# arpitbansal297/Cold-Diffusion-Models

Measured on NVIDIA H100. Metric: training-step images/sec (CelebA-128 deblur UNet, config 3), higher is better.
Workload: dtype tf32

## Files before the change

### cold_diffusion_models_b200/_lib.py

```python
import ctypes as C
import os
import torch

_HERE = os.path.dirname(os.path.abspath(__file__))
LIB_PATH = os.path.join(_HERE, 'csrc', 'libcolddiff.so')
CD_MAX_TAPS = 16
CONV_SIMT, CONV_TC = 0, 1
ACT_NONE, ACT_GELU, ACT_GELU_BWD = 0, 1, 2


class ColdDiffError(RuntimeError):
    pass


if not os.path.exists(LIB_PATH):
    raise ImportError("libcolddiff.so not built (%s); run `python -c 'import __graft_entry__ as g; g.build()'`"
                      % LIB_PATH)
lib = C.CDLL(LIB_PATH)


class ConvSrc(C.Structure):
    _fields_ = [('src', C.c_void_p), ('ld', C.c_int32), ('C', C.c_int32), ('H', C.c_int32), ('W', C.c_int32),
                ('ntaps', C.c_int32), ('dy', C.c_int32 * CD_MAX_TAPS), ('dx', C.c_int32 * CD_MAX_TAPS),
                ('w', C.c_void_p), ('w_per_batch', C.c_int32)]


class ConvDesc(C.Structure):
    _fields_ = [('B', C.c_int32), ('Hg', C.c_int32), ('Wg', C.c_int32), ('sy', C.c_int32), ('sx', C.c_int32),
                ('Cout', C.c_int32), ('nsrc', C.c_int32), ('s', ConvSrc * 2),
                ('out', C.c_void_p), ('out_ld', C.c_int32), ('Ho', C.c_int32), ('Wo', C.c_int32),
                ('oys', C.c_int32), ('oxs', C.c_int32), ('oy0', C.c_int32), ('ox0', C.c_int32),
                ('bias', C.c_void_p), ('resid', C.c_void_p), ('resid_ld', C.c_int32),
                ('act', C.c_int32), ('round_tf32', C.c_int32),
                ('out2', C.c_void_p), ('out2_ld', C.c_int32),
                ('aux', C.c_void_p), ('aux_ld', C.c_int32)]




class RepackJob(C.Structure):
    _fields_ = [('src', C.c_void_p), ('dst', C.c_void_p), ('O', C.c_int32), ('I', C.c_int32), ('KH', C.c_int32), ('KW', C.c_int32),
                ('transposed_conv', C.c_int32), ('mode', C.c_int32), ('ntaps', C.c_int32), ('round_tf32', C.c_int32),
                ('ky', C.c_int32 * CD_MAX_TAPS), ('kx', C.c_int32 * CD_MAX_TAPS), ('block0', C.c_int32), ('nblocks', C.c_int32)]


lib.cd_version.restype = C.c_int
if os.environ.get('COLDDIFF_2CTA') in ('0', '1', '2'):
    lib.cd_conv_tc_set_2cta(int(os.environ['COLDDIFF_2CTA']))
lib.cd_last_error.argtypes = [C.c_char_p, C.c_size_t]
if os.environ.get('COLDDIFF_CONV_TWO_CTAS') in ('0', '64', '128', '192'):
    lib.cd_conv_tc_set_two_ctas(int(os.environ['COLDDIFF_CONV_TWO_CTAS']))
if os.environ.get('COLDDIFF_CONV_HALO') in ('0', '1', '2', '6', '8'):
    lib.cd_conv_tc_set_halo(int(os.environ['COLDDIFF_CONV_HALO']))
if os.environ.get('COLDDIFF_WGRAD_MODE') in ('0', '1', '8'):
    lib.cd_wgrad_tc_set_mode(int(os.environ['COLDDIFF_WGRAD_MODE']))
if os.environ.get('COLDDIFF_2CTA_BN') in ('0', '64', '128', '192'):
    lib.cd_conv_tc_set_2cta_bn(int(os.environ['COLDDIFF_2CTA_BN']))
if os.environ.get('COLDDIFF_CONV_STAGED_EPILOGUE') in ('0', '1', '2', '3'):
    lib.cd_conv_tc_set_staged_epilogue(int(os.environ['COLDDIFF_CONV_STAGED_EPILOGUE']))
if os.environ.get('COLDDIFF_CONV_SIMT_PRELOAD') in ('0', '1'):
    lib.cd_conv_simt_set_preload(int(os.environ['COLDDIFF_CONV_SIMT_PRELOAD']))
if os.environ.get('COLDDIFF_LAYERNORM_MULTI') in ('0', '2', '4'):
    lib.cd_layernorm_set_multi(int(os.environ['COLDDIFF_LAYERNORM_MULTI']))
if os.environ.get('COLDDIFF_LINATTN_STAGED') in ('0', '1'):
    lib.cd_linattn_set_staged(int(os.environ['COLDDIFF_LINATTN_STAGED']))


def _check(rc, what):
    if rc != 0:
        buf = C.create_string_buffer(512)
        lib.cd_last_error(buf, 512)
        raise ColdDiffError("%s failed (%d): %s" % (what, rc, buf.value.decode()))


def stream():
    return C.c_void_p(torch.cuda.current_stream().cuda_stream)


def ptr(t):
    if t is None:
        return C.c_void_p(0)
    return C.c_void_p(t.data_ptr())


_LAUNCHES = {'cd_linattn_context': 2, 'cd_linattn_context_det': 2, 'cd_conv_wgrad': 2, 'cd_time_mlp_fwd': 2, 'cd_time_mlp2_fwd': 2, 'cd_version': 0, 'cd_last_error': 0}
_launch_count = 0


_PROF_SHAPE_ARGS = {'cd_dwconv7_fwd': (2, 3, 4, 5), 'cd_dwconv7_wgrad': (4, 5, 6, 7), 'cd_layernorm_bwd': (6, 7),
                    'cd_layernorm_fwd': (2, 3), 'cd_linattn_context': (2, 3), 'cd_linattn_context_det': (2, 3), 'cd_linattn_bwd_kv': (2, 3)}
_prof = None


def call(name, *args):
    global _launch_count
    _launch_count += _LAUNCHES.get(name, 1)
    if _prof is not None:
        e0, e1 = torch.cuda.Event(enable_timing=True), torch.cuda.Event(enable_timing=True)
        e0.record()
        _check(getattr(lib, name)(*args), name)
        e1.record()
        idx = _PROF_SHAPE_ARGS.get(name)
        if idx:
            name = name + str(tuple(int(getattr(args[i], 'value', args[i])) for i in idx))
        _prof.append((name, e0, e1))
        return
    _check(getattr(lib, name)(*args), name)


def profile_start():
    global _prof
    _prof = []


def profile_stop():
    global _prof
    torch.cuda.synchronize()
    out = {}
    for name, e0, e1 in _prof:
        c, t = out.get(name, (0, 0.0))
        out[name] = (c + 1, t + e0.elapsed_time(e1))
    _prof = None
    return out


def reset_launch_count():
    global _launch_count
    _launch_count = 0


def launch_count():
    return _launch_count


EXPORTS = [
    'cd_version', 'cd_last_error', 'cd_conv_fwd', 'cd_conv_wgrad', 'cd_pack_weight', 'cd_unpack_wgrad',
]
```

### cold_diffusion_models_b200/csrc/conv_tc.cu

```cuda
#include "tc_common.cuh"
#include "conv_epilogue.cuh"

namespace {

constexpr int kTileM = 128;
constexpr int kChunkK = 32;
constexpr int kABytes = kTileM * 128;
constexpr int kThreads = 288;
constexpr int kConsumerWarps = 8;

struct TcParams {
  int B, Hg, Wg;
  int TW, TH, TN;
  int tiles_x, tiles_y, tiles_n, tiles_co, total_tiles;
  int sy, sx;
  int Cout;
  int nsrc;
  int ntaps[2];
  int kchunks[2];
  int wpb[2];
  int8_t dy[2][CD_MAX_TAPS];
  int8_t dx[2][CD_MAX_TAPS];
  float* out; int out_ld; int Ho, Wo; int oys, oxs, oy0, ox0;
  const float* bias;
  const float* resid; int resid_ld;
  int act; int round_tf32;
  float* out2; int out2_ld;
  const float* aux; int aux_ld;
  int nbox[2];
  int8_t boxdx[2][3];
  int8_t boxend[2][3];
  int8_t taporder[2][CD_MAX_TAPS];
  int tapoff[2][CD_MAX_TAPS];
};

__device__ __forceinline__ long long tile_pixel(const TcParams& p, int tile, int m) {
  int mt = tile / p.tiles_co;
  const int tx = mt % p.tiles_x; mt /= p.tiles_x;
  const int ty = mt % p.tiles_y;
  const int tn = mt / p.tiles_y;
  const int gx = tx * p.TW + m % p.TW, gy = ty * p.TH + (m / p.TW) % p.TH, b = tn * p.TN + m / (p.TW * p.TH);
  if (b >= p.B) return -1;
  return (static_cast<long long>(b) * p.Ho + (gy * p.oys + p.oy0)) * p.Wo + (gx * p.oxs + p.ox0);
}

__device__ __forceinline__ void epi_pair(const TcParams& p, long long pix, int col, float v0, float v1) {
  if (col + 1 < p.Cout) {
    float2 v = make_float2(v0, v1);
    if (p.bias) { const float2 b = __ldg(reinterpret_cast<const float2*>(p.bias + col)); v.x += b.x; v.y += b.y; }
    if (p.resid) { const float2 r = *reinterpret_cast<const float2*>(p.resid + pix * p.resid_ld + col); v.x += r.x; v.y += r.y; }
    if (p.out2) *reinterpret_cast<float2*>(p.out2 + pix * p.out2_ld + col) = v;
    if (p.act == CD_ACT_GELU) { v.x = cd_gelu(v.x); v.y = cd_gelu(v.y); }
    else if (p.act == CD_ACT_GELU_BWD) {
      const float2 a = *reinterpret_cast<const float2*>(p.aux + pix * p.aux_ld + col);
      v.x *= cd_gelu_grad(a.x); v.y *= cd_gelu_grad(a.y);
    }
    if (p.round_tf32) { v.x = cd_round_tf32(v.x); v.y = cd_round_tf32(v.y); }
    *reinterpret_cast<float2*>(p.out + pix * p.out_ld + col) = v;
  } else if (col < p.Cout) {
    float v = v0;
    if (p.bias) v += p.bias[col];
    if (p.resid) v += p.resid[pix * p.resid_ld + col];
    if (p.out2) p.out2[pix * p.out2_ld + col] = v;
    if (p.act == CD_ACT_GELU) v = cd_gelu(v);
    else if (p.act == CD_ACT_GELU_BWD) v *= cd_gelu_grad(p.aux[pix * p.aux_ld + col]);
    if (p.round_tf32) v = cd_round_tf32(v);
    p.out[pix * p.out_ld + col] = v;
  }
}

template <int BN, int STAGES, bool STG = false, bool F16 = false, int CTAS = 1, bool PAIR = false>
__global__ void __launch_bounds__(kThreads, CTAS)
conv_tc_kernel(const __grid_constant__ CUtensorMap mapA0, const __grid_constant__ CUtensorMap mapA1,
               const __grid_constant__ CUtensorMap mapB0, const __grid_constant__ CUtensorMap mapB1,
               const TcParams p) {
  constexpr int kBBytes = BN * 128;
  constexpr int kStageBytes = kABytes + kBBytes;
  constexpr int kChunkElems = F16 ? 64 : kChunkK;

  extern __shared__ uint8_t smem_raw[];
  const uint32_t raw_addr = smem_u32(smem_raw);
  const uint32_t pad = (1024u - (raw_addr & 1023u)) & 1023u;
  uint8_t* smem = smem_raw + pad;
  uint64_t* bars = reinterpret_cast<uint64_t*>(smem + STAGES * kStageBytes);
  uint64_t* full_bar = bars;
  uint64_t* empty_bar = bars + STAGES;
  static_assert(2 * STAGES * 8 <= 256, "barrier block is 256 bytes");
  float* epi_stage = reinterpret_cast<float*>(smem + STAGES * kStageBytes + 256);

  const int warp = threadIdx.x >> 5;
  const int lane = threadIdx.x & 31;
  const int wg = threadIdx.x >> 7;

  if (threadIdx.x == 0) {
    for (int i = 0; i < STAGES; ++i) { mbar_init(&full_bar[i], 1); mbar_init(&empty_bar[i], kConsumerWarps * (PAIR ? 2 : 1)); }
    asm volatile("fence.mbarrier_init.release.cluster;" ::: "memory");
  }
  if constexpr (PAIR) cluster_sync(); else __syncthreads();
  const uint32_t rank = PAIR ? cluster_ctarank() : 0;
  const int unit0 = PAIR ? blockIdx.x / 2 : blockIdx.x, ustride = PAIR ? gridDim.x / 2 : gridDim.x;
  const int units = PAIR ? p.tiles_co * ((p.total_tiles / p.tiles_co + 1) / 2) : p.total_tiles;
  auto tile_of = [&](int u) { return PAIR ? ((u / p.tiles_co) * 2 + static_cast<int>(rank)) * p.tiles_co + u % p.tiles_co : u; };

  const int kiters = p.ntaps[0] * p.kchunks[0] + (p.nsrc > 1 ? p.ntaps[1] * p.kchunks[1] : 0);

  if (warp == kConsumerWarps) {
    if (elect_one()) {
      uint32_t stage = 0, ph = 0;
      for (int u = unit0; u < units; u += ustride) {
        const int tile = tile_of(u);
        const int co_t = tile % p.tiles_co;
        int mt = tile / p.tiles_co;
        const int tx = mt % p.tiles_x; mt /= p.tiles_x;
        const int ty = mt % p.tiles_y;
        const int tn = mt / p.tiles_y;
        const int x0 = tx * p.TW * p.sx, y0 = ty * p.TH * p.sy, n0 = tn * p.TN, co0 = co_t * BN;
        for (int s = 0; s < p.nsrc; ++s) {
          const CUtensorMap* mA = s ? &mapA1 : &mapA0;
          const CUtensorMap* mB = s ? &mapB1 : &mapB0;
          const int wbase = p.wpb[s] ? n0 * p.ntaps[s] : 0;
          for (int tap = 0; tap < p.ntaps[s]; ++tap) {
            const int xin = x0 + p.dx[s][tap], yin = y0 + p.dy[s][tap];
            for (int kc = 0; kc < p.kchunks[s]; ++kc) {
              mbar_wait(&empty_bar[stage], ph ^ 1u);
              mbar_expect_tx(&full_bar[stage], kStageBytes);
              const uint32_t sa = smem_u32(smem + stage * kStageBytes);
              tma_load_4d(sa, mA, &full_bar[stage], kc * kChunkElems, xin, yin, n0);
              if constexpr (PAIR)
                tma_load_3d_mc(sa + kABytes + rank * (kBBytes / 2), mB, &full_bar[stage], kc * kChunkElems, co0 + static_cast<int>(rank) * (BN / 2),
                               wbase + tap, static_cast<uint16_t>(3));
              else
                tma_load_3d(sa + kABytes, mB, &full_bar[stage], kc * kChunkElems, co0, wbase + tap);
              if (++stage == STAGES) { stage = 0; ph ^= 1u; }
            }
          }
        }
      }
    }
    __syncwarp();
  } else {
    const int cw = wg;
    const int tid = threadIdx.x & 127;
    const int rl = (tid >> 5) * 16 + (lane >> 2);
    const int q2 = (lane & 3) * 2;
    float acc[BN / 2];
    uint32_t stage = 0, ph = 0;
    auto release = [&](uint32_t st) {
      __syncwarp();
      if (lane == 0) { mbar_arrive(&empty_bar[st]); if constexpr (PAIR) mbar_arrive_cluster(&empty_bar[st], rank ^ 1u); }
    };
    for (int u = unit0; u < units; u += ustride) {
      const int tile = tile_of(u);
      uint32_t prev = 0;
      for (int k = 0; k < kiters; ++k) {
        mbar_wait(&full_bar[stage], ph);
        wgmma_fence();
        const uint32_t sa = smem_u32(smem + stage * kStageBytes);
        const uint64_t da = make_kmajor_sw128_desc(sa + cw * (kABytes / 2));
        const uint64_t db = make_kmajor_sw128_desc(sa + kABytes);
#pragma unroll
        for (int kk = 0; kk < 4; ++kk) {
          if constexpr (F16) wgmma_f16<BN>(acc, da + uint64_t(kk * 2), db + uint64_t(kk * 2), (k | kk) != 0 ? 1u : 0u);
          else wgmma_tf32<BN>(acc, da + uint64_t(kk * 2), db + uint64_t(kk * 2), (k | kk) != 0 ? 1u : 0u);
        }
        wgmma_commit();
        wgmma_wait<1>();
        if (k > 0) release(prev);
        prev = stage;
        if (++stage == STAGES) { stage = 0; ph ^= 1u; }
      }
      wgmma_wait<0>();
      if (kiters > 0) release(prev);

      const int co0 = (tile % p.tiles_co) * BN;
      const long long pix0 = tile_pixel(p, tile, cw * 64 + rl);
      const long long pix1 = tile_pixel(p, tile, cw * 64 + rl + 8);
      if constexpr (STG) {
        float* st = epi_stage + cw * 64 * kEpiStageStride;
        const int bar_id = 1 + cw;
#pragma unroll
        for (int c = 0; c < BN; c += 32) {
          if (co0 + c + 32 <= p.Cout) {
            asm volatile("bar.sync %0, 128;" :: "r"(bar_id) : "memory");
#pragma unroll
            for (int j = c / 8; j < c / 8 + 4; ++j) {
              *reinterpret_cast<float2*>(st + rl * kEpiStageStride + 8 * j - c + q2) = make_float2(acc[4 * j], acc[4 * j + 1]);
              *reinterpret_cast<float2*>(st + (rl + 8) * kEpiStageStride + 8 * j - c + q2) = make_float2(acc[4 * j + 2], acc[4 * j + 3]);
            }
            asm volatile("bar.sync %0, 128;" :: "r"(bar_id) : "memory");
            const int w4 = tid >> 5;
            if (w4 < 2) {
              const int row = w4 * 32 + lane;
              uint32_t r[32];
#pragma unroll
              for (int e = 0; e < 32; ++e) r[e] = __float_as_uint(st[row * kEpiStageStride + e]);
              const long long pix = tile_pixel(p, tile, cw * 64 + row);
              cd_epilogue_staged32(r, st + w4 * 32 * kEpiStageStride, lane, pix < 0 ? 0 : pix, pix >= 0, co0 + c, p);
            }
          } else {
#pragma unroll
            for (int j = c / 8; j < c / 8 + 4; ++j) {
              if (pix0 >= 0) epi_pair(p, pix0, co0 + 8 * j + q2, acc[4 * j], acc[4 * j + 1]);
              if (pix1 >= 0) epi_pair(p, pix1, co0 + 8 * j + q2, acc[4 * j + 2], acc[4 * j + 3]);
            }
          }
        }
      } else {
#pragma unroll
        for (int j = 0; j < BN / 8; ++j) {
          if (pix0 >= 0) epi_pair(p, pix0, co0 + 8 * j + q2, acc[4 * j], acc[4 * j + 1]);
          if (pix1 >= 0) epi_pair(p, pix1, co0 + 8 * j + q2, acc[4 * j + 2], acc[4 * j + 3]);
        }
      }
    }
  }
  if constexpr (PAIR) cluster_sync();
}

constexpr int kRowsTW = 16, kRowsTH = kTileM / kRowsTW;
constexpr int kRowsBoxBytes = kRowsTW * (kRowsTH + 2) * 128;

template <int BN, int ABOXES, int STAGES, int CTAS>
__global__ void __launch_bounds__(kThreads, CTAS)
conv_rows_kernel(const __grid_constant__ CUtensorMap mapA0, const __grid_constant__ CUtensorMap mapA1,
                 const __grid_constant__ CUtensorMap mapB0, const __grid_constant__ CUtensorMap mapB1, const __grid_constant__ TcParams p) {
  constexpr int kBBytes = BN * 128;
  extern __shared__ uint8_t smem_raw[];
  const uint32_t raw_addr = smem_u32(smem_raw);
  uint8_t* smem = smem_raw + ((1024u - (raw_addr & 1023u)) & 1023u);
  uint8_t* abox = smem;
  uint8_t* wtile = smem + ABOXES * kRowsBoxBytes;
  uint64_t* bars = reinterpret_cast<uint64_t*>(wtile + STAGES * kBBytes);
  uint64_t* full_bar = bars;
  uint64_t* empty_bar = bars + STAGES;
  uint64_t* afull = bars + 2 * STAGES;
  uint64_t* aempty = bars + 2 * STAGES + ABOXES;
  static_assert(2 * (STAGES + ABOXES) * 8 <= 256, "barrier block is 256 bytes");
  const int warp = threadIdx.x >> 5, lane = threadIdx.x & 31, wg = threadIdx.x >> 7;
  if (threadIdx.x == 0) {
    for (int i = 0; i < STAGES; ++i) { mbar_init(&full_bar[i], 1); mbar_init(&empty_bar[i], kConsumerWarps); }
    for (int i = 0; i < ABOXES; ++i) { mbar_init(&afull[i], 1); mbar_init(&aempty[i], kConsumerWarps); }
    asm volatile("fence.mbarrier_init.release.cluster;" ::: "memory");
  }
  __syncthreads();

  if (warp == kConsumerWarps) {
    if (elect_one()) {
      uint32_t stage = 0, ph = 0, ai = 0, aph = 0;
      for (int tile = blockIdx.x; tile < p.total_tiles; tile += gridDim.x) {
        const int co0 = (tile % p.tiles_co) * BN;
        int mt = tile / p.tiles_co;
        const int x0 = (mt % p.tiles_x) * kRowsTW; mt /= p.tiles_x;
        const int y0 = (mt % p.tiles_y) * kRowsTH;
        const int n = mt / p.tiles_y;
        for (int s = 0; s < p.nsrc; ++s) {
          const CUtensorMap* mA = s ? &mapA1 : &mapA0;
          const CUtensorMap* mB = s ? &mapB1 : &mapB0;
          for (int kc = 0; kc < p.kchunks[s]; ++kc) {
            for (int b = 0, i = 0; b < p.nbox[s]; ++b) {
              mbar_wait(&aempty[ai], aph ^ 1u);
              mbar_expect_tx(&afull[ai], kRowsBoxBytes);
              tma_load_4d(smem_u32(abox + ai * kRowsBoxBytes), mA, &afull[ai], kc * kChunkK, x0 + p.boxdx[s][b], y0 - 1, n);
              if (++ai == ABOXES) { ai = 0; aph ^= 1u; }
              for (; i < p.boxend[s][b]; ++i) {
                mbar_wait(&empty_bar[stage], ph ^ 1u);
                mbar_expect_tx(&full_bar[stage], kBBytes);
                tma_load_3d(smem_u32(wtile + stage * kBBytes), mB, &full_bar[stage], kc * kChunkK, co0, p.taporder[s][i]);
                if (++stage == STAGES) { stage = 0; ph ^= 1u; }
              }
            }
          }
        }
      }
    }
    __syncwarp();
    return;
  }

  const int tid = threadIdx.x & 127;
  const int rl = (tid >> 5) * 16 + (lane >> 2);
  const int q2 = (lane & 3) * 2;
  auto release = [&](uint64_t* bar) { __syncwarp(); if (lane == 0) mbar_arrive(bar); };
  float acc[BN / 2];
  uint32_t stage = 0, ph = 0, ai = 0, aph = 0;
  for (int tile = blockIdx.x; tile < p.total_tiles; tile += gridDim.x) {
    int k = 0;
    uint32_t prev = 0, prev_a = 0;
    for (int s = 0; s < p.nsrc; ++s) {
      for (int kc = 0; kc < p.kchunks[s]; ++kc) {
        for (int b = 0, i = 0; b < p.nbox[s]; ++b) {
          mbar_wait(&afull[ai], aph);
          const uint32_t abase = smem_u32(abox + ai * kRowsBoxBytes) + wg * (kABytes / 2);
          for (const int i0 = i; i < p.boxend[s][b]; ++i, ++k) {
            mbar_wait(&full_bar[stage], ph);
            wgmma_fence();
            const uint64_t da = make_kmajor_sw128_desc(abase + p.tapoff[s][i]);
            const uint64_t db = make_kmajor_sw128_desc(smem_u32(wtile + stage * kBBytes));
#pragma unroll
            for (int kk = 0; kk < 4; ++kk)
              wgmma_tf32<BN>(acc, da + uint64_t(kk * 2), db + uint64_t(kk * 2), (k | kk) != 0 ? 1u : 0u);
            wgmma_commit();
            wgmma_wait<1>();
            if (k > 0) release(&empty_bar[prev]);
            if (k > 0 && i == i0) release(&aempty[prev_a]);
            prev = stage;
            if (++stage == STAGES) { stage = 0; ph ^= 1u; }
          }
          prev_a = ai;
          if (++ai == ABOXES) { ai = 0; aph ^= 1u; }
        }
      }
    }
    wgmma_wait<0>();
    if (k > 0) { release(&empty_bar[prev]); release(&aempty[prev_a]); }

    const int co0 = (tile % p.tiles_co) * BN;
    int mt = tile / p.tiles_co;
    const int x0 = (mt % p.tiles_x) * kRowsTW; mt /= p.tiles_x;
    const int y0 = (mt % p.tiles_y) * kRowsTH;
    const int n = mt / p.tiles_y;
#pragma unroll
    for (int h = 0; h < 2; ++h) {
      const int m = wg * 64 + rl + 8 * h;
      const int gx = x0 + m % kRowsTW, gy = y0 + m / kRowsTW;
      if (gx >= p.Wg || gy >= p.Hg) continue;
      const long long pix = (static_cast<long long>(n) * p.Ho + (gy * p.oys + p.oy0)) * p.Wo + (gx * p.oxs + p.ox0);
#pragma unroll
      for (int j = 0; j < BN / 8; ++j) epi_pair(p, pix, co0 + 8 * j + q2, acc[4 * j + 2 * h], acc[4 * j + 2 * h + 1]);
    }
  }
}


int g_num_sms = 0;
int g_tf32_map_dtype = 1;


template <int BN, int STAGES, bool STG = false, bool F16 = false, int CTAS = 1, bool PAIR = false>
int launch(const CUtensorMap* maps, const TcParams& p, cudaStream_t st) {
  constexpr size_t smem = size_t(STAGES) * (kABytes + BN * 128) + 1024 + 256 + (STG ? sizeof(float) * 2 * 64 * kEpiStageStride : 0);
  static_assert(smem <= 232448, "dynamic shared memory of one CTA (227 KB)");
  static_assert(CTAS == 1 || 2 * (smem + 1024) <= 233472, "two CTAs per SM must fit the 228 KB of shared memory");
  auto kern = conv_tc_kernel<BN, STAGES, STG, F16, CTAS, PAIR>;
  static bool attr_done = false;
  if (!attr_done) {
    CD_CUDA(cudaFuncSetAttribute(kern, cudaFuncAttributeMaxDynamicSharedMemorySize, (int)smem));
    attr_done = true;
  }
  if constexpr (PAIR) {
    const int units = p.tiles_co * ((p.total_tiles / p.tiles_co + 1) / 2), slots = g_num_sms / 2;
    cudaLaunchConfig_t cfg = {};
    cudaLaunchAttribute attr[1];
    attr[0].id = cudaLaunchAttributeClusterDimension;
    attr[0].val.clusterDim.x = 2; attr[0].val.clusterDim.y = 1; attr[0].val.clusterDim.z = 1;
    cfg.gridDim = dim3(2 * (units < slots ? units : slots)); cfg.blockDim = dim3(kThreads);
    cfg.dynamicSmemBytes = smem; cfg.stream = st; cfg.attrs = attr; cfg.numAttrs = 1;
    CD_CUDA(cudaLaunchKernelEx(&cfg, kern, maps[0], maps[1], maps[2], maps[3], p));
  } else {
    const int slots = g_num_sms * CTAS;
    const int grid = p.total_tiles < slots ? p.total_tiles : slots;
    kern<<<grid, kThreads, smem, st>>>(maps[0], maps[1], maps[2], maps[3], p);
  }
  CD_LAUNCH_CHECK();
  return 0;
}

template <int BN, int ABOXES, int STAGES, int CTAS = 1>
int launch_rows(const CUtensorMap* maps, const TcParams& p, cudaStream_t st) {
  constexpr size_t smem = size_t(ABOXES) * kRowsBoxBytes + size_t(STAGES) * BN * 128 + 1024 + 256;
  static_assert(smem <= 232448, "dynamic shared memory of one CTA (227 KB)");
  static_assert(CTAS == 1 || 2 * (smem + 1024) <= 233472, "two CTAs per SM must fit the 228 KB of shared memory");
  auto kern = conv_rows_kernel<BN, ABOXES, STAGES, CTAS>;
  static bool attr_done = false;
  if (!attr_done) {
    CD_CUDA(cudaFuncSetAttribute(kern, cudaFuncAttributeMaxDynamicSharedMemorySize, (int)smem));
    attr_done = true;
  }
  const int slots = g_num_sms * CTAS;
  const int grid = p.total_tiles < slots ? p.total_tiles : slots;
  kern<<<grid, kThreads, smem, st>>>(maps[0], maps[1], maps[2], maps[3], p);
  CD_LAUNCH_CHECK();
  return 0;
}

}

extern "C" int cd_conv_tc_set_tf32_maps(int enable) { g_tf32_map_dtype = enable ? 1 : 0; return 0; }

static int g_use_2cta = 0;
extern "C" int cd_conv_tc_set_2cta(int mode) { g_use_2cta = mode; return 0; }
static int g_2cta_bn = 0;
extern "C" int cd_conv_tc_set_2cta_bn(int mask) { g_2cta_bn = mask & (128 | 64); return 0; }
static int g_use_halo = 0;
extern "C" int cd_conv_tc_set_halo(int enable) { g_use_halo = enable; return 0; }
static int g_ctas2 = 128 | 64;
extern "C" int cd_conv_tc_set_two_ctas(int mask) { g_ctas2 = mask & (128 | 64); return 0; }
static int g_epi_staged = 0;
constexpr int kStagedMaxKIters = 16;
constexpr int kStagedMidKIters = 48;
extern "C" int cd_conv_tc_set_staged_epilogue(int mode) { g_epi_staged = mode; return 0; }

static double tc_cost(long long m_tiles, int Cout, int BN, int sms, bool pair = false) {
  if (pair) {
    const long long tiles = ((m_tiles + 1) / 2) * (Cout / 256), slots = sms / 2;
    return double((tiles + slots - 1) / slots) * 256.0;
  }
  const long long tiles = m_tiles * ((Cout + BN - 1) / BN);
  const double rate = BN == 256 ? 0.92 : (BN == 128 ? 0.75 : 0.40);
  return double((tiles + sms - 1) / sms) * BN / rate;
}

static int conv_fwd_tc_impl(const CdConvDesc* d, cudaStream_t st, bool f16);
int cd_conv_fwd_tc(const CdConvDesc* d, cudaStream_t st) { return conv_fwd_tc_impl(d, st, false); }

extern "C" int cd_conv_fwd_f16_probe(const CdConvDesc* d, void* stream) {
  CD_REQUIRE(d != nullptr && d->nsrc >= 1 && d->nsrc <= 2, "cd_conv_fwd_f16_probe: bad descriptor");
  return conv_fwd_tc_impl(d, static_cast<cudaStream_t>(stream), true);
}

static int conv_fwd_rows(const CdConvDesc* d, cudaStream_t st, bool by_shape);

static int conv_fwd_tc_impl(const CdConvDesc* d, cudaStream_t st, bool f16) {
  if (!f16 && g_epi_staged == 0) {
    if ((g_use_halo == 0 && !g_use_2cta) || g_use_halo == 1 || g_use_halo == 2 || g_use_halo == 6) {
      const int r = conv_fwd_rows(d, st, g_use_halo == 0);
      if (r <= 0) return r;
    }
  }
  const int chunk_elems = f16 ? 64 : kChunkK;
  const int esz = f16 ? 2 : 4;
  EncodeTiledFn enc = get_encode();
  CD_REQUIRE(enc != nullptr, "cuTensorMapEncodeTiled entry point unavailable");
  if (!g_num_sms) {
    int dev = 0; CD_CUDA(cudaGetDevice(&dev));
    CD_CUDA(cudaDeviceGetAttribute(&g_num_sms, cudaDevAttrMultiProcessorCount, dev));
  }
  CD_REQUIRE(d->nsrc >= 1 && d->nsrc <= 2, "conv_tc: nsrc must be 1 or 2");
  TcParams p{};
  p.B = d->B; p.Hg = d->Hg; p.Wg = d->Wg; p.sy = d->sy; p.sx = d->sx; p.Cout = d->Cout; p.nsrc = d->nsrc;
  if (d->Wg >= 128) {
    CD_REQUIRE(d->Wg % 128 == 0, "conv_tc: Wg >= 128 must be a multiple of 128 (got %d)", d->Wg);
    p.TW = 128; p.TH = 1; p.TN = 1;
  } else {
    CD_REQUIRE(is_pow2(d->Wg), "conv_tc: Wg < 128 must be a power of two (got %d)", d->Wg);
    p.TW = d->Wg;
    int th = 128 / p.TW;
    if (th > d->Hg) th = d->Hg;
    CD_REQUIRE(is_pow2(th) && d->Hg % th == 0, "conv_tc: unsupported Hg %d for Wg %d", d->Hg, d->Wg);
    p.TH = th; p.TN = 128 / (p.TW * p.TH);
  }
  CD_REQUIRE(p.TW * d->sx <= 256 && p.TH * d->sy <= 256, "conv_tc: strided box too large");
  p.tiles_x = d->Wg / p.TW; p.tiles_y = d->Hg / p.TH; p.tiles_n = cd_cdiv(d->B, p.TN);
  int BN = (d->Cout % 256 == 0) ? 256 : (d->Cout > 64 ? 128 : 64);
  int kiters_host = 0;
  for (int s = 0; s < d->nsrc; ++s) kiters_host += d->s[s].ntaps * (d->s[s].C / chunk_elems);
  const bool staged = !f16 &&
                      ( g_epi_staged == 2 || (g_epi_staged == 1 && kiters_host <= kStagedMaxKIters) ||
                      (g_epi_staged == 3 && kiters_host <= kStagedMidKIters));
  bool pair = false;
  const long long mt = static_cast<long long>(p.tiles_x) * p.tiles_y * p.tiles_n;
  if (BN == 256) {
    double best = tc_cost(mt, d->Cout, 256, g_num_sms);
    if (tc_cost(mt, d->Cout, 128, g_num_sms) < best) { BN = 128; best = tc_cost(mt, d->Cout, 128, g_num_sms); }
    if (!f16 && !staged && g_use_2cta && mt >= 2 && (g_use_2cta == 2 || tc_cost(mt, d->Cout, 256, g_num_sms, true) < best)) {
      BN = 256; pair = true;
    }
  } else if (!f16 && !staged && g_use_2cta && (g_2cta_bn & BN) && d->Cout % BN == 0 && (g_use_2cta == 2 || mt >= 2 * g_num_sms)) {
    pair = true;
  }
  p.tiles_co = cd_cdiv(d->Cout, BN);
  p.total_tiles = p.tiles_x * p.tiles_y * p.tiles_n * p.tiles_co;
  p.out = d->out; p.out_ld = d->out_ld; p.Ho = d->Ho; p.Wo = d->Wo;
  p.oys = d->oys; p.oxs = d->oxs; p.oy0 = d->oy0; p.ox0 = d->ox0;
  p.bias = d->bias; p.resid = d->resid; p.resid_ld = d->resid_ld; p.act = d->act; p.round_tf32 = d->round_tf32;
  p.out2 = d->out2; p.out2_ld = d->out2_ld; p.aux = d->aux; p.aux_ld = d->aux_ld;
  CD_REQUIRE(d->act != CD_ACT_GELU_BWD || (d->aux && (reinterpret_cast<uintptr_t>(d->aux) & 15) == 0 && d->aux_ld % 4 == 0), "conv_tc: GELU_BWD needs an aligned aux");
  CD_REQUIRE((reinterpret_cast<uintptr_t>(d->out) & 15) == 0 && d->out_ld % 4 == 0, "conv_tc: out must be 16B aligned");
  CD_REQUIRE(!d->resid || ((reinterpret_cast<uintptr_t>(d->resid) & 15) == 0 && d->resid_ld % 4 == 0), "conv_tc: resid alignment");
  CD_REQUIRE(!d->out2 || ((reinterpret_cast<uintptr_t>(d->out2) & 15) == 0 && d->out2_ld % 4 == 0), "conv_tc: out2 alignment");
  CD_REQUIRE(!d->bias || (reinterpret_cast<uintptr_t>(d->bias) & 15) == 0, "conv_tc: bias alignment");

  CUtensorMap maps[4];
  const CUtensorMapDataType dt = f16 ? CU_TENSOR_MAP_DATA_TYPE_FLOAT16 : (g_tf32_map_dtype ? CU_TENSOR_MAP_DATA_TYPE_TFLOAT32 : CU_TENSOR_MAP_DATA_TYPE_FLOAT32);
  for (int s = 0; s < 2; ++s) {
    const CdConvSrc& cs = d->s[s < d->nsrc ? s : 0];
    CD_REQUIRE(cs.C % chunk_elems == 0 && cs.C > 0, "conv_tc: source channels %d not a multiple of %d", cs.C, chunk_elems);
    CD_REQUIRE(cs.ntaps >= 1 && cs.ntaps <= CD_MAX_TAPS, "conv_tc: bad ntaps");
    CD_REQUIRE((reinterpret_cast<uintptr_t>(cs.src) & 15) == 0 && (cs.ld * esz) % 16 == 0, "conv_tc: src must be 16B aligned");
    CD_REQUIRE((reinterpret_cast<uintptr_t>(cs.w) & 15) == 0, "conv_tc: weights must be 16B aligned");
    CD_REQUIRE(!cs.w_per_batch || p.TN == 1, "conv_tc: per-batch weights need >=128 pixels per image");
    p.ntaps[s] = cs.ntaps; p.kchunks[s] = cs.C / chunk_elems; p.wpb[s] = cs.w_per_batch;
    for (int t = 0; t < cs.ntaps; ++t) { p.dy[s][t] = (int8_t)cs.dy[t]; p.dx[s][t] = (int8_t)cs.dx[t]; }
    {
      cuuint64_t dims[4] = {(cuuint64_t)cs.C, (cuuint64_t)cs.W, (cuuint64_t)cs.H, (cuuint64_t)d->B};
      cuuint64_t strides[3] = {(cuuint64_t)cs.ld * esz, (cuuint64_t)cs.ld * esz * cs.W, (cuuint64_t)cs.ld * esz * cs.W * cs.H};
      cuuint32_t box[4] = {(cuuint32_t)chunk_elems, (cuuint32_t)(p.TW * d->sx), (cuuint32_t)(p.TH * d->sy), (cuuint32_t)p.TN};
      cuuint32_t estr[4] = {1, (cuuint32_t)d->sx, (cuuint32_t)d->sy, 1};
      CUresult r = enc(&maps[s], dt, 4, const_cast<float*>(cs.src), dims, strides, box, estr,
                       CU_TENSOR_MAP_INTERLEAVE_NONE, CU_TENSOR_MAP_SWIZZLE_128B, CU_TENSOR_MAP_L2_PROMOTION_L2_128B,
                       CU_TENSOR_MAP_FLOAT_OOB_FILL_NONE);
      CD_REQUIRE(r == CUDA_SUCCESS, "cuTensorMapEncodeTiled(A%d) failed: %d", s, (int)r);
    }
    {
      const int BNl = BN;
      cuuint64_t dims[3] = {(cuuint64_t)cs.C, (cuuint64_t)d->Cout, (cuuint64_t)cs.ntaps * (cs.w_per_batch ? d->B : 1)};
      cuuint64_t strides[2] = {(cuuint64_t)cs.C * esz, (cuuint64_t)cs.C * esz * d->Cout};
      cuuint32_t box[3] = {(cuuint32_t)chunk_elems, (cuuint32_t)(pair ? BNl / 2 : BNl), 1};
      cuuint32_t estr[3] = {1, 1, 1};
      CUresult r = enc(&maps[2 + s], dt, 3, const_cast<float*>(cs.w), dims, strides, box, estr,
                       CU_TENSOR_MAP_INTERLEAVE_NONE, CU_TENSOR_MAP_SWIZZLE_128B, CU_TENSOR_MAP_L2_PROMOTION_L2_256B,
                       CU_TENSOR_MAP_FLOAT_OOB_FILL_NONE);
      CD_REQUIRE(r == CUDA_SUCCESS, "cuTensorMapEncodeTiled(B%d) failed: %d", s, (int)r);
    }
  }
  if (f16) {
    if (BN == 256) return launch<256, 4, false, true>(maps, p, st);
    if (BN == 128) return launch<128, 6, false, true>(maps, p, st);
    return launch<64, 8, false, true>(maps, p, st);
  }
  if (staged) {
    if (BN == 256) return launch<256, 3, true>(maps, p, st);
    if (BN == 128) return launch<128, 4, true>(maps, p, st);
    return launch<64, 6, true>(maps, p, st);
  }
  if (pair) {
    if (BN == 256) return launch<256, 4, false, false, 1, true>(maps, p, st);
    if (BN == 128) return launch<128, 6, false, false, 1, true>(maps, p, st);
    return launch<64, 8, false, false, 1, true>(maps, p, st);
  }
  const int ctas2 = p.total_tiles > g_num_sms ? g_ctas2 : 0;
  if (BN == 256) return launch<256, 4>(maps, p, st);
  if (BN == 128) return (ctas2 & 128) ? launch<128, 3, false, false, 2>(maps, p, st) : launch<128, 6>(maps, p, st);
  return (ctas2 & 64) ? launch<64, 4, false, false, 2>(maps, p, st) : launch<64, 8>(maps, p, st);
}

static int conv_fwd_rows(const CdConvDesc* d, cudaStream_t st, bool by_shape) {
  if (d->sy != 1 || d->sx != 1 || d->nsrc < 1 || d->nsrc > 2) return 1;
  for (int s = 0; s < d->nsrc; ++s) {
    const CdConvSrc& cs = d->s[s];
    if (cs.w_per_batch || cs.C % kChunkK != 0 || cs.C <= 0 || cs.ntaps < 1 || cs.ntaps > CD_MAX_TAPS) return 1;
    if (cs.W != d->Wg || cs.H != d->Hg) return 1;
    for (int t = 0; t < cs.ntaps; ++t) if (cs.dy[t] < -1 || cs.dy[t] > 1 || cs.dx[t] < -1 || cs.dx[t] > 1) return 1;
    if ((reinterpret_cast<uintptr_t>(cs.src) & 15) || (cs.ld * 4) % 16 || (reinterpret_cast<uintptr_t>(cs.w) & 15)) return 1;
  }
  if ((reinterpret_cast<uintptr_t>(d->out) & 15) || d->out_ld % 4) return 1;
  if (d->resid && ((reinterpret_cast<uintptr_t>(d->resid) & 15) || d->resid_ld % 4)) return 1;
  if (d->out2 && ((reinterpret_cast<uintptr_t>(d->out2) & 15) || d->out2_ld % 4)) return 1;
  if (d->bias && (reinterpret_cast<uintptr_t>(d->bias) & 15)) return 1;
  if (d->act == CD_ACT_GELU_BWD && (!d->aux || (reinterpret_cast<uintptr_t>(d->aux) & 15) || d->aux_ld % 4)) return 1;
  EncodeTiledFn enc = get_encode();
  CD_REQUIRE(enc != nullptr, "cuTensorMapEncodeTiled entry point unavailable");
  if (!g_num_sms) {
    int dev = 0; CD_CUDA(cudaGetDevice(&dev));
    CD_CUDA(cudaDeviceGetAttribute(&g_num_sms, cudaDevAttrMultiProcessorCount, dev));
  }
  TcParams p{};
  p.B = d->B; p.Hg = d->Hg; p.Wg = d->Wg; p.sy = 1; p.sx = 1; p.Cout = d->Cout; p.nsrc = d->nsrc;
  p.TW = kRowsTW; p.TH = kRowsTH; p.TN = 1;
  p.tiles_x = cd_cdiv(d->Wg, kRowsTW); p.tiles_y = cd_cdiv(d->Hg, kRowsTH); p.tiles_n = d->B;
  const int BN = d->Cout > 64 ? 128 : 64;
  p.tiles_co = cd_cdiv(d->Cout, BN);
  p.total_tiles = p.tiles_x * p.tiles_y * p.tiles_n * p.tiles_co;
  if (by_shape && p.total_tiles <= g_num_sms) return 1;
  p.out = d->out; p.out_ld = d->out_ld; p.Ho = d->Ho; p.Wo = d->Wo;
  p.oys = d->oys; p.oxs = d->oxs; p.oy0 = d->oy0; p.ox0 = d->ox0;
  p.bias = d->bias; p.resid = d->resid; p.resid_ld = d->resid_ld; p.act = d->act; p.round_tf32 = d->round_tf32;
  p.out2 = d->out2; p.out2_ld = d->out2_ld; p.aux = d->aux; p.aux_ld = d->aux_ld;
  const CUtensorMapDataType dt = g_tf32_map_dtype ? CU_TENSOR_MAP_DATA_TYPE_TFLOAT32 : CU_TENSOR_MAP_DATA_TYPE_FLOAT32;
  CUtensorMap maps[4];
  for (int s = 0; s < 2; ++s) {
    const CdConvSrc& cs = d->s[s < d->nsrc ? s : 0];
    p.ntaps[s] = cs.ntaps; p.kchunks[s] = cs.C / kChunkK; p.wpb[s] = 0;
    p.nbox[s] = 0;
    int i = 0;
    for (int dx = -1; dx <= 1; ++dx) {
      const int i0 = i;
      for (int t = 0; t < cs.ntaps; ++t)
        if (cs.dx[t] == dx) { p.taporder[s][i] = (int8_t)t; p.tapoff[s][i] = (cs.dy[t] + 1) * kRowsTW * 128; ++i; }
      if (i > i0) { p.boxdx[s][p.nbox[s]] = (int8_t)dx; p.boxend[s][p.nbox[s]] = (int8_t)i; ++p.nbox[s]; }
    }
    if (s == 0 && cs.ntaps < 3 * p.nbox[0]) return 1;
    for (int t = 0; t < cs.ntaps; ++t) { p.dy[s][t] = (int8_t)cs.dy[t]; p.dx[s][t] = (int8_t)cs.dx[t]; }
    {
      cuuint64_t dims[4] = {(cuuint64_t)cs.C, (cuuint64_t)cs.W, (cuuint64_t)cs.H, (cuuint64_t)d->B};
      cuuint64_t strides[3] = {(cuuint64_t)cs.ld * 4, (cuuint64_t)cs.ld * 4 * cs.W, (cuuint64_t)cs.ld * 4 * cs.W * cs.H};
      cuuint32_t box[4] = {(cuuint32_t)kChunkK, (cuuint32_t)kRowsTW, (cuuint32_t)(kRowsTH + 2), 1};
      cuuint32_t estr[4] = {1, 1, 1, 1};
      CUresult r = enc(&maps[s], dt, 4, const_cast<float*>(cs.src), dims, strides, box, estr,
                       CU_TENSOR_MAP_INTERLEAVE_NONE, CU_TENSOR_MAP_SWIZZLE_128B, CU_TENSOR_MAP_L2_PROMOTION_L2_128B,
                       CU_TENSOR_MAP_FLOAT_OOB_FILL_NONE);
      CD_REQUIRE(r == CUDA_SUCCESS, "cuTensorMapEncodeTiled(rows A%d) failed: %d", s, (int)r);
    }
    {
      cuuint64_t dims[3] = {(cuuint64_t)cs.C, (cuuint64_t)d->Cout, (cuuint64_t)cs.ntaps};
      cuuint64_t strides[2] = {(cuuint64_t)cs.C * 4, (cuuint64_t)cs.C * 4 * d->Cout};
      cuuint32_t box[3] = {(cuuint32_t)kChunkK, (cuuint32_t)BN, 1};
      cuuint32_t estr[3] = {1, 1, 1};
      CUresult r = enc(&maps[2 + s], dt, 3, const_cast<float*>(cs.w), dims, strides, box, estr,
                       CU_TENSOR_MAP_INTERLEAVE_NONE, CU_TENSOR_MAP_SWIZZLE_128B, CU_TENSOR_MAP_L2_PROMOTION_L2_256B,
                       CU_TENSOR_MAP_FLOAT_OOB_FILL_NONE);
      CD_REQUIRE(r == CUDA_SUCCESS, "cuTensorMapEncodeTiled(rows B%d) failed: %d", s, (int)r);
    }
  }
  const int ctas2 = p.total_tiles > g_num_sms ? g_ctas2 : 0;
  if (BN == 128) return (ctas2 & 128) ? launch_rows<128, 3, 3, 2>(maps, p, st) : launch_rows<128, 6, 4>(maps, p, st);
  return (ctas2 & 64) ? launch_rows<64, 3, 6, 2>(maps, p, st) : launch_rows<64, 6, 8>(maps, p, st);
}
```

Baseline: 619.9.

## Add CTA-pair weight multicast to rows conv and split producer warps

Adds an optional two-CTA cluster mode to the row-tiled implicit-GEMM conv kernel. Each CTA loads half of the weight tile and multicasts it to its partner, and the empty barriers are arrived on across the cluster. Separately, the producer role is split across two warps, one issuing activation box loads and one issuing weight loads, so the two TMA streams no longer serialize. The pair mode is opt-in through new halo settings 4/5. The extra warp raises the thread count per CTA on the default path and may add register pressure at two CTAs per SM.

```diff
diff --git a/cold_diffusion_models_b200/_lib.py b/cold_diffusion_models_b200/_lib.py
--- a/cold_diffusion_models_b200/_lib.py
+++ b/cold_diffusion_models_b200/_lib.py
@@ -50,7 +50,7 @@
 lib.cd_last_error.argtypes = [C.c_char_p, C.c_size_t]
 if os.environ.get('COLDDIFF_CONV_TWO_CTAS') in ('0', '64', '128', '192'):
     lib.cd_conv_tc_set_two_ctas(int(os.environ['COLDDIFF_CONV_TWO_CTAS']))
-if os.environ.get('COLDDIFF_CONV_HALO') in ('0', '1', '2', '6', '8'):
+if os.environ.get('COLDDIFF_CONV_HALO') in ('0', '1', '2', '4', '5', '6', '8'):
     lib.cd_conv_tc_set_halo(int(os.environ['COLDDIFF_CONV_HALO']))
 if os.environ.get('COLDDIFF_WGRAD_MODE') in ('0', '1', '8'):
     lib.cd_wgrad_tc_set_mode(int(os.environ['COLDDIFF_WGRAD_MODE']))
diff --git a/cold_diffusion_models_b200/csrc/conv_tc.cu b/cold_diffusion_models_b200/csrc/conv_tc.cu
--- a/cold_diffusion_models_b200/csrc/conv_tc.cu
+++ b/cold_diffusion_models_b200/csrc/conv_tc.cu
@@ -219,9 +219,29 @@
 
 constexpr int kRowsTW = 16, kRowsTH = kTileM / kRowsTW;
 constexpr int kRowsBoxBytes = kRowsTW * (kRowsTH + 2) * 128;
-
-template <int BN, int ABOXES, int STAGES, int CTAS>
-__global__ void __launch_bounds__(kThreads, CTAS)
+constexpr int kRowsThreads = kThreads + 32;
+
+struct RowsTile { int x0, y0, n, co0; };
+template <bool PAIR>
+__device__ __forceinline__ RowsTile rows_tile(const TcParams& p, int u, uint32_t rank, int BN) {
+  RowsTile t;
+  t.co0 = (u % p.tiles_co) * BN;
+  int mt = u / p.tiles_co;
+  if constexpr (PAIR) {
+    mt = 2 * mt + static_cast<int>(rank);
+    t.y0 = (mt % p.tiles_y) * kRowsTH; mt /= p.tiles_y;
+    t.x0 = (mt % p.tiles_x) * kRowsTW;
+    t.n = mt / p.tiles_x;
+  } else {
+    t.x0 = (mt % p.tiles_x) * kRowsTW; mt /= p.tiles_x;
+    t.y0 = (mt % p.tiles_y) * kRowsTH;
+    t.n = mt / p.tiles_y;
+  }
+  return t;
+}
+
+template <int BN, int ABOXES, int STAGES, int CTAS, bool PAIR = false>
+__global__ void __launch_bounds__(kRowsThreads, CTAS)
 conv_rows_kernel(const __grid_constant__ CUtensorMap mapA0, const __grid_constant__ CUtensorMap mapA1,
                  const __grid_constant__ CUtensorMap mapB0, const __grid_constant__ CUtensorMap mapB1, const __grid_constant__ TcParams p) {
   constexpr int kBBytes = BN * 128;
@@ -238,42 +258,51 @@
   static_assert(2 * (STAGES + ABOXES) * 8 <= 256, "barrier block is 256 bytes");
   const int warp = threadIdx.x >> 5, lane = threadIdx.x & 31, wg = threadIdx.x >> 7;
   if (threadIdx.x == 0) {
-    for (int i = 0; i < STAGES; ++i) { mbar_init(&full_bar[i], 1); mbar_init(&empty_bar[i], kConsumerWarps); }
+    for (int i = 0; i < STAGES; ++i) { mbar_init(&full_bar[i], 1); mbar_init(&empty_bar[i], kConsumerWarps * (PAIR ? 2 : 1)); }
     for (int i = 0; i < ABOXES; ++i) { mbar_init(&afull[i], 1); mbar_init(&aempty[i], kConsumerWarps); }
     asm volatile("fence.mbarrier_init.release.cluster;" ::: "memory");
   }
-  __syncthreads();
-
-  if (warp == kConsumerWarps) {
+  if constexpr (PAIR) cluster_sync(); else __syncthreads();
+  const uint32_t rank = PAIR ? cluster_ctarank() : 0;
+  const int unit0 = PAIR ? blockIdx.x / 2 : blockIdx.x, ustride = PAIR ? gridDim.x / 2 : gridDim.x;
+  const int units = PAIR ? p.tiles_co * ((p.total_tiles / p.tiles_co + 1) / 2) : p.total_tiles;
+
+  if (warp >= kConsumerWarps) {
+    const bool box_warp = warp == kConsumerWarps;
     if (elect_one()) {
       uint32_t stage = 0, ph = 0, ai = 0, aph = 0;
-      for (int tile = blockIdx.x; tile < p.total_tiles; tile += gridDim.x) {
-        const int co0 = (tile % p.tiles_co) * BN;
-        int mt = tile / p.tiles_co;
-        const int x0 = (mt % p.tiles_x) * kRowsTW; mt /= p.tiles_x;
-        const int y0 = (mt % p.tiles_y) * kRowsTH;
-        const int n = mt / p.tiles_y;
+      for (int u = unit0; u < units; u += ustride) {
+        const RowsTile t = rows_tile<PAIR>(p, u, rank, BN);
+        const int co0 = t.co0, x0 = t.x0, y0 = t.y0, n = t.n;
         for (int s = 0; s < p.nsrc; ++s) {
           const CUtensorMap* mA = s ? &mapA1 : &mapA0;
           const CUtensorMap* mB = s ? &mapB1 : &mapB0;
           for (int kc = 0; kc < p.kchunks[s]; ++kc) {
-            for (int b = 0, i = 0; b < p.nbox[s]; ++b) {
-              mbar_wait(&aempty[ai], aph ^ 1u);
-              mbar_expect_tx(&afull[ai], kRowsBoxBytes);
-              tma_load_4d(smem_u32(abox + ai * kRowsBoxBytes), mA, &afull[ai], kc * kChunkK, x0 + p.boxdx[s][b], y0 - 1, n);
-              if (++ai == ABOXES) { ai = 0; aph ^= 1u; }
-              for (; i < p.boxend[s][b]; ++i) {
-                mbar_wait(&empty_bar[stage], ph ^ 1u);
-                mbar_expect_tx(&full_bar[stage], kBBytes);
+            if (box_warp) {
+              for (int b = 0; b < p.nbox[s]; ++b) {
+                mbar_wait(&aempty[ai], aph ^ 1u);
+                mbar_expect_tx(&afull[ai], kRowsBoxBytes);
+                tma_load_4d(smem_u32(abox + ai * kRowsBoxBytes), mA, &afull[ai], kc * kChunkK, x0 + p.boxdx[s][b], y0 - 1, n);
+                if (++ai == ABOXES) { ai = 0; aph ^= 1u; }
+              }
+              continue;
+            }
+            for (int i = 0; i < p.boxend[s][p.nbox[s] - 1]; ++i) {
+              mbar_wait(&empty_bar[stage], ph ^ 1u);
+              mbar_expect_tx(&full_bar[stage], kBBytes);
+              if constexpr (PAIR)
+                tma_load_3d_mc(smem_u32(wtile + stage * kBBytes + rank * (kBBytes / 2)), mB, &full_bar[stage], kc * kChunkK,
+                               co0 + static_cast<int>(rank) * (BN / 2), p.taporder[s][i], static_cast<uint16_t>(3));
+              else
                 tma_load_3d(smem_u32(wtile + stage * kBBytes), mB, &full_bar[stage], kc * kChunkK, co0, p.taporder[s][i]);
-                if (++stage == STAGES) { stage = 0; ph ^= 1u; }
-              }
+              if (++stage == STAGES) { stage = 0; ph ^= 1u; }
             }
           }
         }
       }
     }
     __syncwarp();
+    if constexpr (PAIR) cluster_sync();
     return;
   }
 
@@ -281,9 +310,13 @@
   const int rl = (tid >> 5) * 16 + (lane >> 2);
   const int q2 = (lane & 3) * 2;
   auto release = [&](uint64_t* bar) { __syncwarp(); if (lane == 0) mbar_arrive(bar); };
+  auto release_w = [&](uint64_t* bar) {
+    __syncwarp();
+    if (lane == 0) { mbar_arrive(bar); if constexpr (PAIR) mbar_arrive_cluster(bar, rank ^ 1u); }
+  };
   float acc[BN / 2];
   uint32_t stage = 0, ph = 0, ai = 0, aph = 0;
-  for (int tile = blockIdx.x; tile < p.total_tiles; tile += gridDim.x) {
+  for (int u = unit0; u < units; u += ustride) {
     int k = 0;
     uint32_t prev = 0, prev_a = 0;
     for (int s = 0; s < p.nsrc; ++s) {
@@ -301,7 +334,7 @@
               wgmma_tf32<BN>(acc, da + uint64_t(kk * 2), db + uint64_t(kk * 2), (k | kk) != 0 ? 1u : 0u);
             wgmma_commit();
             wgmma_wait<1>();
-            if (k > 0) release(&empty_bar[prev]);
+            if (k > 0) release_w(&empty_bar[prev]);
             if (k > 0 && i == i0) release(&aempty[prev_a]);
             prev = stage;
             if (++stage == STAGES) { stage = 0; ph ^= 1u; }
@@ -312,23 +345,21 @@
       }
     }
     wgmma_wait<0>();
-    if (k > 0) { release(&empty_bar[prev]); release(&aempty[prev_a]); }
-
-    const int co0 = (tile % p.tiles_co) * BN;
-    int mt = tile / p.tiles_co;
-    const int x0 = (mt % p.tiles_x) * kRowsTW; mt /= p.tiles_x;
-    const int y0 = (mt % p.tiles_y) * kRowsTH;
-    const int n = mt / p.tiles_y;
+    if (k > 0) { release_w(&empty_bar[prev]); release(&aempty[prev_a]); }
+
+    const RowsTile t = rows_tile<PAIR>(p, u, rank, BN);
+    if (PAIR && t.n >= p.B) continue;
 #pragma unroll
     for (int h = 0; h < 2; ++h) {
       const int m = wg * 64 + rl + 8 * h;
-      const int gx = x0 + m % kRowsTW, gy = y0 + m / kRowsTW;
+      const int gx = t.x0 + m % kRowsTW, gy = t.y0 + m / kRowsTW;
       if (gx >= p.Wg || gy >= p.Hg) continue;
-      const long long pix = (static_cast<long long>(n) * p.Ho + (gy * p.oys + p.oy0)) * p.Wo + (gx * p.oxs + p.ox0);
-#pragma unroll
-      for (int j = 0; j < BN / 8; ++j) epi_pair(p, pix, co0 + 8 * j + q2, acc[4 * j + 2 * h], acc[4 * j + 2 * h + 1]);
-    }
-  }
+      const long long pix = (static_cast<long long>(t.n) * p.Ho + (gy * p.oys + p.oy0)) * p.Wo + (gx * p.oxs + p.ox0);
+#pragma unroll
+      for (int j = 0; j < BN / 8; ++j) epi_pair(p, pix, t.co0 + 8 * j + q2, acc[4 * j + 2 * h], acc[4 * j + 2 * h + 1]);
+    }
+  }
+  if constexpr (PAIR) cluster_sync();
 }
 
 
@@ -365,20 +396,38 @@
   return 0;
 }
 
-template <int BN, int ABOXES, int STAGES, int CTAS = 1>
+template <int BN, int ABOXES, int STAGES, int CTAS = 1, bool PAIR = false>
 int launch_rows(const CUtensorMap* maps, const TcParams& p, cudaStream_t st) {
   constexpr size_t smem = size_t(ABOXES) * kRowsBoxBytes + size_t(STAGES) * BN * 128 + 1024 + 256;
   static_assert(smem <= 232448, "dynamic shared memory of one CTA (227 KB)");
   static_assert(CTAS == 1 || 2 * (smem + 1024) <= 233472, "two CTAs per SM must fit the 228 KB of shared memory");
-  auto kern = conv_rows_kernel<BN, ABOXES, STAGES, CTAS>;
+  static_assert(!PAIR || CTAS == 2, "the CTA pair runs at two CTAs per SM");
+  auto kern = conv_rows_kernel<BN, ABOXES, STAGES, CTAS, PAIR>;
   static bool attr_done = false;
   if (!attr_done) {
     CD_CUDA(cudaFuncSetAttribute(kern, cudaFuncAttributeMaxDynamicSharedMemorySize, (int)smem));
     attr_done = true;
   }
-  const int slots = g_num_sms * CTAS;
-  const int grid = p.total_tiles < slots ? p.total_tiles : slots;
-  kern<<<grid, kThreads, smem, st>>>(maps[0], maps[1], maps[2], maps[3], p);
+  if constexpr (PAIR) {
+    cudaLaunchConfig_t cfg = {};
+    cudaLaunchAttribute attr[1];
+    attr[0].id = cudaLaunchAttributeClusterDimension;
+    attr[0].val.clusterDim.x = 2; attr[0].val.clusterDim.y = 1; attr[0].val.clusterDim.z = 1;
+    cfg.blockDim = dim3(kRowsThreads); cfg.dynamicSmemBytes = smem; cfg.stream = st; cfg.attrs = attr; cfg.numAttrs = 1;
+    static int clusters = 0;
+    if (!clusters) {
+      cfg.gridDim = dim3(2 * g_num_sms);
+      CD_CUDA(cudaOccupancyMaxActiveClusters(&clusters, kern, &cfg));
+      CD_REQUIRE(clusters > 0, "conv_rows pair kernel: no cluster of two CTAs fits an SM pair");
+    }
+    const int units = p.tiles_co * ((p.total_tiles / p.tiles_co + 1) / 2);
+    cfg.gridDim = dim3(2 * (units < clusters ? units : clusters));
+    CD_CUDA(cudaLaunchKernelEx(&cfg, kern, maps[0], maps[1], maps[2], maps[3], p));
+  } else {
+    const int slots = g_num_sms * CTAS;
+    const int grid = p.total_tiles < slots ? p.total_tiles : slots;
+    kern<<<grid, kRowsThreads, smem, st>>>(maps[0], maps[1], maps[2], maps[3], p);
+  }
   CD_LAUNCH_CHECK();
   return 0;
 }
@@ -392,6 +441,7 @@
 static int g_2cta_bn = 0;
 extern "C" int cd_conv_tc_set_2cta_bn(int mask) { g_2cta_bn = mask & (128 | 64); return 0; }
 static int g_use_halo = 0;
+constexpr int kHaloRowsPair = 4, kHaloRowsPairAlways = 5;
 extern "C" int cd_conv_tc_set_halo(int enable) { g_use_halo = enable; return 0; }
 static int g_ctas2 = 128 | 64;
 extern "C" int cd_conv_tc_set_two_ctas(int mask) { g_ctas2 = mask & (128 | 64); return 0; }
@@ -422,7 +472,8 @@
 
 static int conv_fwd_tc_impl(const CdConvDesc* d, cudaStream_t st, bool f16) {
   if (!f16 && g_epi_staged == 0) {
-    if ((g_use_halo == 0 && !g_use_2cta) || g_use_halo == 1 || g_use_halo == 2 || g_use_halo == 6) {
+    if ((g_use_halo == 0 && !g_use_2cta) || g_use_halo == 1 || g_use_halo == 2 || g_use_halo == 6 ||
+        g_use_halo == kHaloRowsPair || g_use_halo == kHaloRowsPairAlways) {
       const int r = conv_fwd_rows(d, st, g_use_halo == 0);
       if (r <= 0) return r;
     }
@@ -562,6 +613,9 @@
   p.tiles_co = cd_cdiv(d->Cout, BN);
   p.total_tiles = p.tiles_x * p.tiles_y * p.tiles_n * p.tiles_co;
   if (by_shape && p.total_tiles <= g_num_sms) return 1;
+  const bool pair_always = g_use_halo == kHaloRowsPairAlways;
+  const int ctas2 = (p.total_tiles > g_num_sms || pair_always) ? g_ctas2 : 0;
+  const bool pair = (pair_always || g_use_halo == kHaloRowsPair) && (ctas2 & BN);
   p.out = d->out; p.out_ld = d->out_ld; p.Ho = d->Ho; p.Wo = d->Wo;
   p.oys = d->oys; p.oxs = d->oxs; p.oy0 = d->oy0; p.ox0 = d->ox0;
   p.bias = d->bias; p.resid = d->resid; p.resid_ld = d->resid_ld; p.act = d->act; p.round_tf32 = d->round_tf32;
@@ -594,7 +648,7 @@
     {
       cuuint64_t dims[3] = {(cuuint64_t)cs.C, (cuuint64_t)d->Cout, (cuuint64_t)cs.ntaps};
       cuuint64_t strides[2] = {(cuuint64_t)cs.C * 4, (cuuint64_t)cs.C * 4 * d->Cout};
-      cuuint32_t box[3] = {(cuuint32_t)kChunkK, (cuuint32_t)BN, 1};
+      cuuint32_t box[3] = {(cuuint32_t)kChunkK, (cuuint32_t)(pair ? BN / 2 : BN), 1};
       cuuint32_t estr[3] = {1, 1, 1};
       CUresult r = enc(&maps[2 + s], dt, 3, const_cast<float*>(cs.w), dims, strides, box, estr,
                        CU_TENSOR_MAP_INTERLEAVE_NONE, CU_TENSOR_MAP_SWIZZLE_128B, CU_TENSOR_MAP_L2_PROMOTION_L2_256B,
@@ -602,7 +656,7 @@
       CD_REQUIRE(r == CUDA_SUCCESS, "cuTensorMapEncodeTiled(rows B%d) failed: %d", s, (int)r);
     }
   }
-  const int ctas2 = p.total_tiles > g_num_sms ? g_ctas2 : 0;
+  if (pair) return BN == 128 ? launch_rows<128, 3, 3, 2, true>(maps, p, st) : launch_rows<64, 3, 6, 2, true>(maps, p, st);
   if (BN == 128) return (ctas2 & 128) ? launch_rows<128, 3, 3, 2>(maps, p, st) : launch_rows<128, 6, 4>(maps, p, st);
   return (ctas2 & 64) ? launch_rows<64, 3, 6, 2>(maps, p, st) : launch_rows<64, 6, 8>(maps, p, st);
 }
```

Result: no change. 622.8 (median of 6 runs) (+0.5%).
